# vibhatha/cylon

Hardware: AMD Instinct MI355X
Metric: rows/sec distributed inner-join, 1B×1B int64 keys, at 1/2/4/8 MI355X (higher is better)
Workload: dtype int64 keys / float64 payload; 1 GPU; model=distributed inner join (hash), int64 key + 3 float64 cols, global_batch=1000000000, seq_len=4, parallelism=dp1 (local join), rows_per_relation=1000000000, output_rows=1010151446, key_range=990000000

## Files before the change

cylon_amd/csrc/cylon/kernels/kernel_decls.inc:

```
void row_partition_hash(const ColView *cols, int ncols, int64_t n, uint32_t *h, void *stream);
void hash_to_partition(const uint32_t *h, int64_t n, uint32_t nparts, uint32_t *pid,
                       int64_t *counts, void *stream);
int64_t partition_positions_workspace(int64_t n, uint32_t nparts);
void partition_positions(const uint32_t *pid, int64_t n, uint32_t nparts, int64_t *block_hist,
                         int64_t *pos, int64_t *counts, void *stream);
void scatter_columns(const ColView *in, const MutColView *out, int ncols, const int64_t *pos,
                     int64_t n, void *stream);
void scatter_var_lengths(const ColView &in, const int64_t *pos, int64_t n, int64_t *out_lens
                            , void *stream);
void scatter_var_bytes(const ColView &in, const int64_t *pos, int64_t n,
                       const int64_t *out_offsets, uint8_t *out_bytes, uint8_t *out_valid
                          , void *stream);
void gather_columns(const ColView *in, const MutColView *out, int ncols, const int64_t *idx,
                    int64_t m, void *stream);
void str_to_i64(const ColView &c, int64_t n, int64_t *out, uint8_t *ok, void *stream);
void str_to_f64(const ColView &c, int64_t n, double *out, uint8_t *ok, void *stream);
void i64_to_str_lengths(const int64_t *v, const uint8_t *valid, int64_t n, int64_t *lens, void *stream);
void i64_to_str_write(const int64_t *v, const uint8_t *valid, int64_t n, const int64_t *offs, uint8_t *bytes,
                      void *stream);
void select_var_lengths(const ColView &a, const ColView &b, int b_bcast, const uint8_t *cond, int64_t n,
                        int64_t *out_lens, void *stream);
void select_var_bytes(const ColView &a, const ColView &b, int b_bcast, const uint8_t *cond, int64_t n,
                      const int64_t *out_offsets, uint8_t *out_bytes, uint8_t *out_valid, void *stream);
void gather_var_lengths(const ColView &in, const int64_t *idx, int64_t m, int64_t *out_lens
// ... 106 lines not shown
                    uint64_t *hash = nullptr, bool inv = false);
void words_to_bytes(const int64_t *const *words, int64_t n, int L, uint8_t *bytes, void *stream,
                    const uint64_t *hash = nullptr);
void words_mismatch(const int64_t *const *a, const int64_t *const *b, int W, const uint8_t *va, const uint8_t *vb,
                    int64_t n, uint8_t *bad, int64_t *nbad, void *stream);
void var_to_words(const uint8_t *bytes, const int64_t *offs, int64_t n, int W, int64_t *const *words,
                  uint64_t *hash, int64_t *lens, uint64_t *h2, void *stream, bool text = false,
                  unsigned int *nul = nullptr);
void padded_text_lens(const int64_t *const *words, const uint64_t *hash, int64_t n, int W, int64_t *lens,
                      void *stream);
void words_to_var(const int64_t *const *words, const uint64_t *hash, const int64_t *lens, const int64_t *out_offs,
                  int64_t n, int W, uint8_t *bytes, void *stream, bool text = false);
void var_hash2(const uint8_t *bytes, const int64_t *offs, int64_t n, uint64_t *h1, uint64_t *h2, void *stream,
               bool pack_row = false);
void radix_part_sample(const int64_t *keys, int64_t n, int bits, int64_t stride, uint32_t *hist,
                       const NarrowKeys *nk, void *stream);
void radix_sort_msd_first_pass(const int64_t *keys, int64_t n, int hr, int db1, int db2, uint64_t key_xor,
                               uint64_t sub, int64_t *out, int64_t slot, int64_t *ws, int64_t *counts,
                               unsigned int *overflow, void *stream);
void radix_sort_msd_second_pass(const int64_t *images, int64_t n, int hr, int db1, int db2, uint64_t sub,
                                const int64_t *first_ws, const int64_t *first_counts, int64_t first_slot, int64_t *out,
                                int64_t slot, int64_t *ws, int64_t *counts, unsigned int *overflow, void *stream);
int64_t seg_sort_capacity();
void seg_sort_local(const int64_t *in, const int64_t *counts, int64_t slot, int64_t nparts, const int64_t *out_offs,
                    uint64_t sub, int local_bits, uint64_t out_xor, int64_t *out, void *stream);
void radix_range_rows_pass(const int64_t *keys, int64_t n, uint64_t flip, uint64_t mn, int rshift, int shift,
                           int digit_bits, const uint8_t *const *in, uint8_t *const *out, const int *widths, int ncols,
                           int64_t *ws, void *stream);
void radix_range_part_offsets(const int64_t *keys, int64_t n, uint64_t flip, uint64_t mn, int rshift, int bits,
                              int64_t *offs, void *stream);
int64_t range_join_max_rows();
int range_join_max_shift();
void range_join_count(const int64_t *lkeys, const int64_t *loffs, const int64_t *rkeys, const int64_t *roffs,
                      int64_t nparts, uint64_t flip, uint64_t mn, int rshift, int64_t *counts, int *overflow,
                      void *stream);
void range_join_write(const int64_t *lkeys, const int64_t *loffs, const int64_t *rkeys, const int64_t *roffs,
                      int64_t nparts, uint64_t flip, uint64_t mn, int rshift, const int64_t *out_offs,
                      const uint8_t *const *lin, uint8_t *const *lout, const int *lw, int nlc,
                      const uint8_t *const *rin, uint8_t *const *rout, const int *rw, int nrc, void *stream);
int64_t radix_join_capacity(const int *widths, const uint8_t *const *in, int n, bool match_flags = false, int key_bytes = 8);
constexpr int kRJItemWords = 5;
constexpr int kRJItemPDefer = 1, kRJItemBDefer = 2, kRJItemPEmit = 4, kRJItemBEmit = 8;
struct RJSplit {
  const int64_t *items = nullptr;
  int64_t nitems = 0;
  const uint8_t *skip = nullptr;
  uint8_t *gprobe = nullptr;
  uint8_t *gbuild = nullptr;
};
void radix_join_count(const int64_t *pkeys, const int64_t *poffs, const int64_t *bkeys, const int64_t *boffs,
                      int64_t nparts, int64_t cap, int64_t *counts, int *overflow, void *stream, int64_t pstride = 1,
                      int outer = 0, int64_t pslot = 0, int64_t bslot = 0, const RJSplit *split = nullptr,
                      const int64_t *narrow_base = nullptr);
void radix_join_write(const int64_t *pkeys, const int64_t *poffs, const int64_t *bkeys, const int64_t *boffs,
                      int64_t nparts, int64_t cap, const int64_t *out_offs, const uint8_t *const *pin,
                      uint8_t *const *pout, const int *pw, int npc, const uint8_t *const *bin, uint8_t *const *bout,
                      const int *bw, int nbc, void *stream, int64_t *cursor = nullptr, int64_t out_cap = 0,
                      int *overflow = nullptr, int pkey = -1, int outer = 0, uint8_t *ppres = nullptr,
                      uint8_t *bpres = nullptr, int64_t pslot = 0, int64_t bslot = 0, const RJSplit *split = nullptr,
                      const int64_t *narrow_base = nullptr);
int64_t distinct_estimate_workspace();
double distinct_estimate(const int64_t *keys, int64_t n, uint32_t *regs, void *stream);
int64_t radix_groupby_slots(int nacc);
int radix_groupby_planes(int nacc);
void radix_groupby_agg(const int64_t *keys, const int64_t *offs, int64_t nparts, const RGAccDesc *acc, int nacc,
                       int64_t *okeys, uint64_t *oacc, int64_t n, int64_t *gcount, int *overflow, void *stream);
int64_t radix_quantile_capacity();
void radix_groupby_quantile(const int64_t *keys, const uint8_t *vals, int vwidth, int vkind, const uint8_t *valid,
                            const int64_t *offs, int64_t nparts, int bits, double q, int64_t *okeys, uint64_t *oq,
                            uint64_t *ovalid, int64_t *gcount, int *overflow, void *stream, uint64_t *fused = nullptr,
                            int64_t n = 0);
void radix_groupby_pack(const int64_t *offs, const int64_t *goff, int64_t nparts, const int64_t *okeys,
                        const uint64_t *oacc, int64_t n, int nacc, int64_t *keys_out, uint64_t *acc_out,
                        int64_t ngroups, void *stream);
void radix_sort_rows_pass(const int64_t *keys, int64_t n, int shift, int digit_bits, const uint8_t *const *in,
                          uint8_t *const *out, const int *widths, int ncols, int64_t *ws, void *stream,
                          uint64_t key_xor, uint64_t digit_flip = 0, bool tiles_prescanned = false,
                          const uint16_t *nd_in = nullptr, uint16_t *nd_out = nullptr, int nd_shift = 0,
                          int nd_bits = 0, uint64_t sub = 0, const SortLbArgs *lb = nullptr);
bool radix_sort_lb_eligible(int64_t n, int ncols, const int *widths, const int *dbits, int npass, void *stream);
int64_t radix_sort_lb_workspace(int64_t n);
SortLbArgs radix_sort_lb_args(int64_t *ws, int64_t n, int pass, int npass, void *stream);
bool radix_sort_lb_failed(const int64_t *ws, void *stream);
int64_t radix_sort_prehist_workspace(int64_t n);
uint64_t radix_sort_prehist(const int64_t *keys, int64_t n, uint64_t flip, int64_t *pre_ws, void *stream,
                            uint64_t *img_min = nullptr, uint64_t *img_max = nullptr);
void radix_sort_prehist_fold(const int64_t *pre_ws, int64_t n, int db, int64_t *ws, void *stream, uint64_t sub = 0);
uint64_t varying_bits(const uint64_t *keys, int64_t n, int64_t *ws2, void *stream);
uint64_t sort_keys_varying_bits(const ColView &col, int64_t n, bool desc, uint64_t *out, int64_t *ws2, void *stream);
void setop_row_hash_tiles(const ColView *lcols, const ColView *rcols, int ncols, int64_t nl, int64_t n, uint64_t *h,
                          int bits, int digit_bits, uint16_t *th, void *colsets, void *stream);
int64_t setop_colsets_bytes();
int64_t setop_rows_per_part();
void setop_dedup(const uint64_t *ph, const int64_t *prow, const int64_t *offs, int64_t nparts, int64_t nl, int op,
                 bool keep_last, const ColView *lcols, const ColView *rcols, int ncols, uint8_t *mask, int64_t *exc,
                 int *bad, void *stream);
int64_t semi_join_capacity();
int64_t semi_join_slice_rows();
void semi_join_mark(const int64_t *rkeys, const int64_t *roffs, const int64_t *lkeys, const int64_t *lrow,
                    const int64_t *loffs, int64_t nparts, int anti, uint8_t *mask, int64_t *matched, int *overflow,
                    const int64_t *ipart, const int64_t *islice, int64_t nitems, int64_t *dkeys, int64_t *dmeta,
                    void *stream);
int topk_digit_bits();
int64_t topk_state_words();
int64_t topk_workspace();
void topk_scan(const ColView &col, int64_t n, bool desc, int64_t *ws, void *stream);
void topk_start(int64_t *ws, int64_t k, int ihi, int rhi, void *stream);
void topk_hist(const ColView &col, int64_t n, bool desc, int64_t *ws, int src, int db, void *stream);
void topk_pick(int64_t *ws, int src, int db, void *stream);
void topk_collect(const ColView &col, int64_t n, bool desc, int64_t *ws, uint64_t *sure_img, int64_t *sure_row,
                  int64_t sure_cap, uint64_t *cand_img, int64_t *cand_row, int64_t cand_cap, void *stream);
void narrow_i64(const int64_t *in, int64_t n, int64_t base, uint32_t *out, void *stream);
void widen_u32(const uint32_t *in, int64_t n, int64_t base, int64_t *out, void *stream);
// ... 90 lines not shown
```

cylon_amd/csrc/cylon/kernels/lds_join.hip:

```cpp
#include "radix_common.hpp"

namespace cylon {
namespace hip {

constexpr int kRJBuckets = 4096;

int64_t radix_join_capacity(const int *widths, const uint8_t *const *in, int n, bool match_flags, int key_bytes) {
  int64_t row = key_bytes + 2 + (match_flags ? 1 : 0);
  for (int q = 0; q < n; ++q)
    if (in[q]) row += widths[q];
  int64_t cap = kRJRowArea / row;
  cap = std::min<int64_t>(cap, kRJMaxRows);
  return cap & ~int64_t(7);
}

__device__ __forceinline__ uint32_t rj_bucket(int64_t k) {
  return (uint32_t)hashing::fmix64((uint64_t)k) & (kRJBuckets - 1);
}
__device__ __forceinline__ uint32_t rj_bucket(uint32_t k) { return hashing::fmix32(k) & (kRJBuckets - 1); }

constexpr int kRJRowsPerThread = kRJMaxRows / kRJThreads;
static_assert(kRJRowsPerThread * kRJThreads == kRJMaxRows, "build rows per thread");
constexpr int kRJProbeRounds = 1;

// ... 460 lines not shown
          if (pc.n > MAXP) {
            const int64_t lo = s0 + (int64_t)u * kWave + owner;
            for (int q = MAXP; q < pc.n; ++q)
              stw<W8>(pc.out[q], o, pc.width[q], q == pkey ? kw : ldw<W8>(pc.in[q], lo, pc.width[q]));
          }
          if ((OJ & kOJProbe) && r < 0) {
#pragma unroll
            for (int q = 0; q < MAXB + 1; ++q)
              if (q < bo.n) stw<W8>(bo.out[q], o, bo.width[q], 0ull);
            for (int q = MAXB + 1; q < bo.n; ++q) stw<W8>(bo.out[q], o, bo.width[q], 0ull);
          } else {
#pragma unroll
            for (int q = 0; q < MAXB + 1; ++q)
              if (q < bo.n)
                stw<W8>(bo.out[q], o, bo.width[q],
                        bo.lds_off[q] < 0 ? kw : ldw<W8>(area + bo.lds_off[q], r, bo.width[q]));
            for (int q = MAXB + 1; q < bo.n; ++q)
              stw<W8>(bo.out[q], o, bo.width[q],
                      bo.lds_off[q] < 0 ? kw : ldw<W8>(area + bo.lds_off[q], r, bo.width[q]));
          }
          if (OJ & kOJProbe) bpres[o] = r >= 0 ? 1 : 0;
          if (OJ & kOJBuild) ppres[o] = 1;
        }
      }
      base += wsum;
    }
    if ((OJ & kOJBuild) && !bdefer) {
      __syncthreads();
      int64_t at = ubase;
      for (int i0 = 0; i0 < nr; i0 += kRJThreads) {
        const int i = i0 + (int)threadIdx.x;
        const uint32_t um = (i < nr && !flg[i]) ? 1u : 0u;
        const uint32_t ex = rp_block_exscan<kRJWaves>(um, wtot);
        uint32_t tot = 0;
#pragma unroll
        for (int w = 0; w < kRJWaves; ++w) tot += wtot[w];
        if (um) {
          const int64_t o = at + ex;
          const int r = perm[i];
          const uint64_t kw = key_value(skeys[i]);
          for (int q = 0; q < pc.n; ++q) stw<W8>(pc.out[q], o, pc.width[q], q == pkey ? kw : 0ull);
          for (int q = 0; q < bo.n; ++q)
            stw<W8>(bo.out[q], o, bo.width[q], bo.lds_off[q] < 0 ? kw : ldw<W8>(area + bo.lds_off[q], r, bo.width[q]));
          ppres[o] = 0;
          if (OJ & kOJProbe) bpres[o] = 1;
        }
        at += tot;
        __syncthreads();
      }
    }
  }
}

static int rj_grid(int64_t nparts) { return (int)std::min<int64_t>(nparts, kNumCUs * 8); }

void radix_join_count(const int64_t *pkeys, const int64_t *poffs, const int64_t *bkeys, const int64_t *boffs,
                      int64_t nparts, int64_t cap, int64_t *counts, int *overflow, void *stream, int64_t pstride,
                      int outer, int64_t pslot, int64_t bslot, const RJSplit *split, const int64_t *narrow_base) {
  CYLON_CHECK(cap > 0 && cap <= kRJMaxRows, Code::Invalid, "radix join capacity " << cap);
  CYLON_CHECK(pstride >= 1, Code::Invalid, "partition stride " << pstride);
  CYLON_CHECK(outer >= 0 && outer <= 3, Code::Invalid, "radix join outer mode " << outer);
  hipStream_t s = as_stream(stream);
  HIP_CHECK(hipMemsetAsync(overflow, 0, sizeof(int), s));
  const int64_t *items = split ? split->items : nullptr;
  const int64_t nitems = items ? split->nitems : 0;
  const uint8_t *skip = split ? split->skip : nullptr;
  const int64_t nsample = items ? nitems : (nparts + pstride - 1) / pstride;
  if (nsample == 0) return;
  const dim3 grid((unsigned)std::max<int64_t>(1, std::min<int64_t>(nsample, kNumCUs * 12)));
  switch (outer) {
    case 0:
      if (narrow_base)
        hipLaunchKernelGGL((k_rj_count<0, true>), grid, dim3(kRCThreads), 0, s, pkeys, poffs, bkeys, boffs, nparts,
                           (int)cap, pstride, counts, overflow, pslot, bslot, items, nitems, skip);
      else
        hipLaunchKernelGGL((k_rj_count<0, false>), grid, dim3(kRCThreads), 0, s, pkeys, poffs, bkeys, boffs, nparts,
                           (int)cap, pstride, counts, overflow, pslot, bslot, items, nitems, skip);
      break;
    case 1:
      if (narrow_base)
        hipLaunchKernelGGL((k_rj_count<1, true>), grid, dim3(kRCThreads), 0, s, pkeys, poffs, bkeys, boffs, nparts,
                           (int)cap, pstride, counts, overflow, pslot, bslot, items, nitems, skip);
      else
        hipLaunchKernelGGL((k_rj_count<1, false>), grid, dim3(kRCThreads), 0, s, pkeys, poffs, bkeys, boffs, nparts,
                           (int)cap, pstride, counts, overflow, pslot, bslot, items, nitems, skip);
      break;
    case 2:
      if (narrow_base)
        hipLaunchKernelGGL((k_rj_count<2, true>), grid, dim3(kRCThreads), 0, s, pkeys, poffs, bkeys, boffs, nparts,
                           (int)cap, pstride, counts, overflow, pslot, bslot, items, nitems, skip);
      else
        hipLaunchKernelGGL((k_rj_count<2, false>), grid, dim3(kRCThreads), 0, s, pkeys, poffs, bkeys, boffs, nparts,
                           (int)cap, pstride, counts, overflow, pslot, bslot, items, nitems, skip);
      break;
    default:
      if (narrow_base)
        hipLaunchKernelGGL((k_rj_count<3, true>), grid, dim3(kRCThreads), 0, s, pkeys, poffs, bkeys, boffs, nparts,
                           (int)cap, pstride, counts, overflow, pslot, bslot, items, nitems, skip);
      else
        hipLaunchKernelGGL((k_rj_count<3, false>), grid, dim3(kRCThreads), 0, s, pkeys, poffs, bkeys, boffs, nparts,
                           (int)cap, pstride, counts, overflow, pslot, bslot, items, nitems, skip);
  }
  HIP_LAUNCH_CHECK();
}

template <bool W8, bool DMA, int OJ>
static void rj_write_launch(dim3 grid, hipStream_t s, const int64_t *pk, const int64_t *poffs, const int64_t *bk,
                            const int64_t *boffs, int64_t nparts, int cap, const int64_t *out_offs, const ColSet &pc,
                            const ColSet &bs, const BuildOut &bo, unsigned long long *cur, int64_t out_cap,
                            int *overflow, int pkey, uint8_t *ppres, uint8_t *bpres,
                            int64_t pslot, int64_t bslot, const RJSplit &sp, const int64_t *nb) {
  if (nb)
    hipLaunchKernelGGL((k_rj_write<4, 3, W8, DMA, OJ, true>), grid, dim3(kRJThreads), 0, s, pk, poffs, bk, boffs, nparts,
                       cap, out_offs, pc, bs, bo, cur, out_cap, overflow, pkey, ppres, bpres, pslot, bslot, sp.items,
                       sp.nitems, sp.skip, sp.gprobe, sp.gbuild, nb);
  else
    hipLaunchKernelGGL((k_rj_write<4, 3, W8, DMA, OJ, false>), grid, dim3(kRJThreads), 0, s, pk, poffs, bk, boffs,
                       nparts, cap, out_offs, pc, bs, bo, cur, out_cap, overflow, pkey, ppres, bpres, pslot, bslot,
                       sp.items, sp.nitems, sp.skip, sp.gprobe, sp.gbuild, nb);
}

void radix_join_write(const int64_t *pkeys, const int64_t *poffs, const int64_t *bkeys, const int64_t *boffs,
                      int64_t nparts, int64_t cap, const int64_t *out_offs, const uint8_t *const *pin,
                      uint8_t *const *pout, const int *pw, int npc, const uint8_t *const *bin, uint8_t *const *bout,
                      const int *bw, int nbc, void *stream, int64_t *cursor, int64_t out_cap, int *overflow, int pkey,
                      int outer, uint8_t *ppres, uint8_t *bpres, int64_t pslot, int64_t bslot,
                      const RJSplit *split, const int64_t *narrow_base) {
  CYLON_CHECK(pkey >= -1 && pkey < npc, Code::Invalid, "radix join probe key column " << pkey);
  CYLON_CHECK(npc <= kMaxFusedCols && nbc <= kMaxFusedCols, Code::Invalid, "too many columns");
  CYLON_CHECK(out_offs != nullptr || (cursor != nullptr && overflow != nullptr), Code::Invalid,
              "radix join write: needs partition offsets or an output cursor");
  CYLON_CHECK(outer >= 0 && outer <= 3, Code::Invalid, "radix join outer mode " << outer);
  CYLON_CHECK(!(outer & kOJProbe) || bpres, Code::Invalid, "radix join: probe-preserving mode needs build presence");
  CYLON_CHECK(!(outer & kOJBuild) || ppres, Code::Invalid, "radix join: build-preserving mode needs probe presence");
  const RJSplit sp = split ? *split : RJSplit{};
  CYLON_CHECK(sp.nitems == 0 || (out_offs == nullptr && sp.items), Code::Invalid,
              "radix join write: split items need the cursor mode");
  if (sp.nitems + nparts == 0) return;
  const int kbytes = narrow_base ? 4 : 8;
  CYLON_CHECK(cap > 0 && cap <= radix_join_capacity(bw, bin, nbc, outer & kOJBuild, kbytes), Code::Invalid,
              "radix join capacity " << cap);
  ColSet pc, bs;
  BuildOut bo;
  pc.n = npc;
  bs.n = 0;
  bo.n = nbc;
  bool w8 = true;
  for (int q = 0; q < kMaxFusedCols; ++q) {
    pc.in[q] = q < npc ? pin[q] : nullptr;
    pc.out[q] = q < npc ? pout[q] : nullptr;
    pc.width[q] = q < npc ? pw[q] : 8;
    bs.in[q] = nullptr;
    bs.out[q] = nullptr;
    bs.width[q] = 8;
    bo.out[q] = q < nbc ? bout[q] : nullptr;
    bo.width[q] = q < nbc ? bw[q] : 8;
    bo.lds_off[q] = -1;
    if (q < npc) w8 &= pw[q] == 8;
    if (q < nbc) w8 &= bw[q] == 8;
  }
  int64_t off = (kbytes + 2) * cap;
  for (int q = 0; q < nbc; ++q)
    if (bin[q]) {
      bo.lds_off[q] = (int)off;
      off += cap * bw[q];
      bs.in[bs.n] = bin[q];
      bs.width[bs.n++] = bw[q];
    }
  bo.match_off = (int)off;
  if (outer & kOJBuild) off += cap;
  CYLON_CHECK(off <= kRJRowArea, Code::Invalid, "radix join LDS rows " << off);
  hipStream_t s = as_stream(stream);
  unsigned long long *cur = reinterpret_cast<unsigned long long *>(cursor);
  const dim3 grid(rj_grid(nparts + sp.nitems));
  const bool dma = w8;
  const int ci = (int)cap;
#define RJW(W8_, DMA_, OJ_)                                                                                        \
  rj_write_launch<W8_, DMA_, OJ_>(grid, s, pkeys, poffs, bkeys, boffs, nparts, ci, out_offs, pc, bs, bo, cur, out_cap, \
                                  overflow, pkey, ppres, bpres, pslot, bslot, sp, narrow_base)
  if (outer == 0) {
    if (dma) RJW(true, true, 0);
    else if (w8) RJW(true, false, 0);
    else RJW(false, false, 0);
  } else if (outer == 1) {
    if (dma) RJW(true, true, 1);
    else RJW(false, false, 1);
  } else if (outer == 2) {
    if (dma) RJW(true, true, 2);
    else RJW(false, false, 2);
  } else {
    if (dma) RJW(true, true, 3);
    else RJW(false, false, 3);
  }
#undef RJW
  HIP_LAUNCH_CHECK();
}


void preload_lds_join() { preload_code(reinterpret_cast<const void *>(&(k_rj_count<0, false>))); }

}
}
```

cylon_amd/csrc/cylon/ops/join_radix.cpp:

```cpp
#include "cylon/knobs.hpp"
#include <algorithm>
#include <array>
#include <cmath>
#include <cstdlib>

#include "join_internal.hpp"
#include "radix_sizing.hpp"
#include "../trace.hpp"

namespace cylon {
namespace ops {

int64_t radix_join_min_rows() {
  return knobs::Int("RADIX_JOIN_MIN_ROWS", int64_t(1) << 22);
}

bool radix_eligible(const TablePtr &t) {
  int slots = 1;
  for (const auto &c : t->columns()) {
    const int w = c.type.width();
    if (c.is_var() || c.type.kind() == ValueKind::FIXED_BYTES || !(w == 1 || w == 2 || w == 4 || w == 8) ||
        c.data.element_size() != w)
      return false;
    slots += 1 + (c.nullable() ? 1 : 0);
// ... 189 lines not shown
  p.cap4 = capacity(4);
  p.cap8 = capacity(8);
  p.narrow = narrow;
  p.split_rows = split_rows_of(p.cap());
  const int64_t nb = std::min(p.nl, p.nr);
  if (pre_bits >= 0) {
    p.set_bits(pre_bits);
    return p;
  }
  p.set_bits(radix_extra_bits(sizing::partition_bits(nb, p.cap())));
  if (p.narrow && p.bits == 0) {
    p = p.without_narrowing();
    p.set_bits(radix_extra_bits(sizing::partition_bits(nb, p.cap())));
  }
  return p;
}

struct RadixJoinIn {
  const Exec &ex;
  const TablePtr &left, &right;
  const JoinConfig &cfg;
  JoinSink *sink;
  const PrePartition *pre;
};

struct Narrowing {
  at::Tensor bad;
  at::Tensor base_src;
  hip::NarrowKeys nk;
};

struct SkewMasks {
  at::Tensor bcnt, pcnt, heavy, mid, sums;
  int64_t cap = 0;
};

static SkewMasks skew_masks(const RadixJoinPlan &plan, const RadixSide &Bs, const RadixSide &Ps) {
  SkewMasks k;
  k.cap = plan.cap();
  const int64_t nparts = plan.nparts, np_rows = plan.build_left ? plan.nr : plan.nl;
  k.bcnt = part_counts(Bs, nparts);
  k.pcnt = part_counts(Ps, nparts);
  k.heavy = at::logical_or(k.bcnt > plan.split_rows, k.pcnt > 2 * plan.pch);
  k.mid = at::logical_and(k.heavy.logical_not(),
                          at::logical_or(k.pcnt > 4 * (np_rows + nparts - 1) / nparts + 1024, k.bcnt > 4 * plan.bmean + 1024));
  k.sums = at::stack({k.heavy.sum(), k.mid.sum()});
  return k;
}

struct Partitioned {
  RadixSide L, R;
  bool released = false;
  SkewMasks sk;
};

static bool fail(bool released, const char *why) {
  CYLON_CHECK(!released, Code::ExecutionError,
              "radix join with a released (retain = false) input could not complete: " << why);
  return false;
}

static void drop_slots_of_skewed_sides(const RadixJoinIn &in, const RadixJoinPlan &plan, const at::Tensor &lk,
                                       const at::Tensor &rk, const hip::NarrowKeys *nkp, int64_t &sl, int64_t &sr) {
  const Exec &ex = in.ex;
  auto sample = [&](const at::Tensor &k, int64_t rows, at::Tensor &h, int64_t &stride) {
    stride = std::max<int64_t>(1, rows >> 20);
    h = at::empty({plan.nparts}, ex.opts(at::kInt));
    hip::radix_part_sample(ptr<int64_t>(k), rows, plan.bits, stride, reinterpret_cast<uint32_t *>(h.data_ptr<int>()),
                           nkp, ex.stream);
  };
  at::Tensor hl, hr;
  int64_t stl = 1, str = 1;
  sample(lk, plan.nl, hl, stl);
  sample(rk, plan.nr, hr, str);
  at::Tensor mx = at::stack({hl.max(), hr.max()}).cpu();
  auto hot = [&](int64_t m, int64_t rows, int64_t stride) {
    const double mean = (double)((rows + stride - 1) / stride) / (double)plan.nparts;
    return (double)m > 4.0 * mean + 32.0;
  };
  if (sl && hot(mx[0].item<int>(), plan.nl, stl)) sl = 0;
  if (sr && hot(mx[1].item<int>(), plan.nr, str)) sr = 0;
  if (!sl || !sr) trace::add_counter("join.radix.sampled_skew_sides", (sl ? 0 : 1) + (sr ? 0 : 1));
}

static Partitioned partition_sides(const RadixJoinIn &in, RadixJoinPlan &plan, at::Tensor &lk, at::Tensor &rk,
                                   const Narrowing &nw) {
  const Exec &ex = in.ex;
  const TablePtr &left = in.left, &right = in.right;
  const int bits = plan.bits;
  Partitioned out;
  RadixSide &L = out.L, &R = out.R;
  const bool rel_l = !left->IsRetain() && !in.sink, rel_r = !right->IsRetain() && !in.sink;
  const bool narrow = plan.narrow;
  at::Tensor r_outside;
  if (rel_l && narrow) {
    auto mm = at::aminmax(rk);
    const at::Tensor base = nw.base_src - (int64_t(1) << 31);
    r_outside = at::logical_or(std::get<0>(mm) < base, (std::get<1>(mm) - base) > (int64_t)0xffffffffll).to(at::kInt);
  }
  auto release_if_done = [&](const TablePtr &t, at::Tensor &key, const RadixSide &s, const at::Tensor *outside) {
    at::Tensor z = at::zeros({1}, ex.opts(at::kInt));
    std::vector<at::Tensor> flags{s.slot ? s.overflow.slice(0, 0, 1) : z, narrow ? nw.bad : z};
    if (outside) flags.push_back(outside->defined() ? outside->reshape({1}) : z);
    if (at::cat(flags).sum().item<int>() != 0) return;
    t->ReleaseIfNotRetained();
    key = at::Tensor();
    trace::add_counter("join.radix.released_inputs", 1);
    out.released = true;
  };
  CYLON_PHASE("join.radix.partition", ex.device);
  const hip::NarrowKeys *nkp = narrow ? &nw.nk : nullptr;
  const bool slot_on = knobs::Flag("RJ_SLOT", true);
  int64_t sl = slot_on ? plan.slot_l : 0, sr = slot_on ? plan.slot_r : 0;
  if ((sl || sr) && std::max(plan.nl, plan.nr) >= (int64_t(1) << 24) && (!in.sink || in.sink->sample_skew))
    drop_slots_of_skewed_sides(in, plan, lk, rk, nkp, sl, sr);
  L = radix_partition(ex, left, lk, bits, nullptr, sl, nkp);
  if (rel_l) release_if_done(left, lk, L, &r_outside);
  R = radix_partition(ex, right, rk, bits, nullptr, sr, nkp);
  if (rel_r) release_if_done(right, rk, R, nullptr);
  if (!(L.slot || R.slot || narrow)) return out;
  at::Tensor z = at::zeros({}, ex.opts(at::kInt));
  out.sk = skew_masks(plan, plan.build_left ? L : R, plan.build_left ? R : L);
  at::Tensor f = at::cat({at::stack({L.slot ? L.overflow[0] : z, R.slot ? R.overflow[0] : z,
                                     narrow ? nw.bad[0] : z}).to(at::kLong),
                          out.sk.sums}).cpu();
  bool redo = f[2].item<int64_t>() != 0;
  if (redo) {
    trace::add_counter("join.radix.narrow_fallback", 1);
    plan = plan.without_narrowing();
    nkp = nullptr;
    L = radix_partition(ex, left, lk, bits, nullptr, slot_on ? plan.slot_l : 0);
    R = radix_partition(ex, right, rk, bits, nullptr, slot_on ? plan.slot_r : 0);
    if (L.slot || R.slot)
      f = at::stack({L.slot ? L.overflow[0] : z, R.slot ? R.overflow[0] : z, z}).to(at::kLong).cpu();
  }
  if (f[0].item<int64_t>()) {
    trace::add_counter("join.radix.slot_overflow", 1);
    L = radix_partition(ex, left, lk, bits, nullptr, 0, nkp);
    redo = true;
  }
  if (f[1].item<int64_t>()) {
    trace::add_counter("join.radix.slot_overflow", 1);
    R = radix_partition(ex, right, rk, bits, nullptr, 0, nkp);
    redo = true;
  }
  if (redo) out.sk = SkewMasks();
  else out.sk.sums = f.slice(0, 3, 5);
  trace::add_counter("join.radix.slot_sides", (L.slot ? 1 : 0) + (R.slot ? 1 : 0));
  if (plan.narrow) trace::add_counter("join.radix.narrow_keys", 1);
  return out;
}

struct SplitWork {
  int64_t nheavy = 0, nmid = 0, nitems = 0, nemits = 0;
  int64_t emit_bound = 0;
  at::Tensor skip, skip_sample, items_d, emits_d, gprobe, gbuild, mid_items;
  hip::RJSplit main, emit;
};

static void split_items(const RadixJoinPlan &plan, const int64_t *h, int64_t nheavy, std::vector<int64_t> &items,
                        std::vector<int64_t> &emits, int64_t &emit_bound) {
  const int oj = plan.oj;
  const int64_t split_rows = plan.split_rows, pch = plan.pch;
  std::vector<std::array<int64_t, hip::kRJItemWords>> work;
  for (int64_t i = 0; i < nheavy; ++i) {
    const int64_t lb0 = h[4 * i], nl0 = h[4 * i + 1], rb0 = h[4 * i + 2], nr0 = h[4 * i + 3];
    const int64_t nbc = std::max<int64_t>(1, (nr0 + split_rows - 1) / split_rows);
    const int64_t npc = nl0 > 2 * pch ? (nl0 + pch - 1) / pch : 1;
    const bool pdef = (oj & 1) && nbc > 1, bdef = (oj & 2) && npc > 1;
    const int64_t fl = (pdef ? hip::kRJItemPDefer : 0) | (bdef ? hip::kRJItemBDefer : 0);
    for (int64_t bc = 0; bc < nbc; ++bc)
      for (int64_t pc = 0; pc < npc; ++pc) {
        const int64_t b0 = nr0 * bc / nbc, b1 = nr0 * (bc + 1) / nbc, p0 = nl0 * pc / npc, p1 = nl0 * (pc + 1) / npc;
        if (b1 > b0 || p1 > p0) work.push_back({lb0 + p0, p1 - p0, rb0 + b0, b1 - b0, fl});
      }
    if (pdef) {
      for (int64_t pc = 0; pc < npc; ++pc)
        emits.insert(emits.end(), {lb0 + nl0 * pc / npc, nl0 * (pc + 1) / npc - nl0 * pc / npc, 0, 0,
                                   (int64_t)hip::kRJItemPEmit});
      emit_bound += nl0;
    }
    if (bdef) {
      for (int64_t bc = 0; bc < nbc; ++bc)
// ... 187 lines not shown
      for (const auto &col : t->columns())
        proto.emplace_back(prefix + col.name, col.type, 0, col.data, at::Tensor(),
                           col.nullable() || may_null ? col.data : at::Tensor());
    };
    add(in.left, in.cfg.GetLeftTablePrefix(), left_may_null(in.cfg.GetType()));
    add(in.right, in.cfg.GetRightTablePrefix(), right_may_null(in.cfg.GetType()));
    o.off = in.sink->reserve(ex, rows, proto);
    o.lcols.assign(in.sink->cols.begin(), in.sink->cols.begin() + nlc);
    o.rcols.assign(in.sink->cols.begin() + nlc, in.sink->cols.end());
  } else {
    auto add = [&](const TablePtr &t, const std::string &prefix, int shared_col, std::vector<Column> &cols) {
      for (int c = 0; c < t->Columns(); ++c)
        cols.push_back(make_fixed_column(prefix + t->column(c).name, t->column(c).type, c == shared_col ? 0 : rows,
                                         ex.device, t->column(c).nullable()));
    };
    add(in.left, in.cfg.GetLeftTablePrefix(), share.on && plan.build_left ? share.kl : -1, o.lcols);
    add(in.right, in.cfg.GetRightTablePrefix(), share.on && !plan.build_left ? share.kr : -1, o.rcols);
  }
  auto word_outs = [&](const RadixSide &sd) {
    std::vector<at::Tensor> w;
    for (size_t i = 0; i < sd.vwords.size(); ++i) w.push_back(ex.empty_i64(std::max<int64_t>(rows, 1)));
    return w;
  };
  o.lwords = word_outs(pt.L);
  o.rwords = word_outs(pt.R);
  if (plan.oj & 2) o.ppres = ex.empty_u8(std::max<int64_t>(rows, 1));
  if (plan.oj & 1) o.bpres = ex.empty_u8(std::max<int64_t>(rows, 1));
}

static void write_output(const RadixJoinIn &in, const JoinLaunch &jl, const Partitioned &pt, const SharedKey &share,
                         const SplitWork &w, JoinOutput &o, int64_t rows, const int64_t *offs, int64_t *cursor) {
  const RadixJoinPlan &plan = jl.plan;
  const RadixSide &P = jl.P, &B = jl.B;
  const bool build_left = plan.build_left;
  RadixCols lc = radix_cols(in.left, &pt.L, &o.lcols, o.off, &o.lwords);
  RadixCols rc = radix_cols(in.right, &pt.R, &o.rcols, o.off, &o.rwords);
  RadixCols &pc = build_left ? rc : lc, &bc = build_left ? lc : rc;
  if (share.on) {
    const TablePtr &bt = build_left ? in.left : in.right;
    const int bkc = build_left ? share.kl : share.kr;
    int q = 0;
    for (int c = 0; c < bkc; ++c) q += 1 + (bt->column(c).nullable() && B.vwords.empty());
    bc.in.erase(bc.in.begin() + q);
    bc.out.erase(bc.out.begin() + q);
    bc.w.erase(bc.w.begin() + q);
  }
  int pkey = -1;
  for (size_t q = 0; q < pc.in.size(); ++q)
    if (!pc.in[q]) {
      pc.in[q] = reinterpret_cast<const uint8_t *>(P.keys.data_ptr());
      if (pkey < 0) pkey = (int)q;
    }
  auto launch = [&](int64_t np, const int64_t *out_offs, const hip::RJSplit &sp) {
    hip::radix_join_write(kptr(P.keys), ptr<int64_t>(P.offs), kptr(B.keys), ptr<int64_t>(B.offs), np, plan.cap(),
                          out_offs, pc.in.data(), pc.out.data(), pc.w.data(), (int)pc.in.size(), bc.in.data(),
                          bc.out.data(), bc.w.data(), (int)bc.in.size(), jl.ex.stream, cursor, rows,
                          jl.overflow.data_ptr<int>(), pkey, plan.oj,
                          o.ppres.defined() ? o.ppres.data_ptr<uint8_t>() : nullptr,
                          o.bpres.defined() ? o.bpres.data_ptr<uint8_t>() : nullptr, P.slot, B.slot, &sp, jl.nbase);
  };
  launch(plan.nparts, offs, w.main);
  if (w.nemits > 0) launch(0, nullptr, w.emit);
}

static bool allocate_and_write(const RadixJoinIn &in, const JoinLaunch &jl, const Partitioned &pt,
                               const SharedKey &share, const SplitWork &w, JoinOutput &o) {
  const Exec &ex = in.ex;
  JoinSink *sink = in.sink;
  const at::Tensor &overflow = jl.overflow;
  int64_t &m = o.m;
  if (o.stride == 1) {
    allocate_output(in, jl.plan, pt, share, m, o);
    if (m > 0) write_output(in, jl, pt, share, w, o, m, ptr<int64_t>(o.out_offs), nullptr);
    return true;
  }
  at::Tensor cursor = at::zeros({1}, ex.opts(at::kLong));
  overflow.zero_();
  allocate_output(in, jl.plan, pt, share, o.alloc, o);
  write_output(in, jl, pt, share, w, o, o.alloc, nullptr, ptr<int64_t>(cursor));
  at::Tensor res = at::cat({cursor, overflow.to(at::kLong)}).cpu();
  m = res[0].item<int64_t>();
  const int64_t flags = res[1].item<int64_t>();
  if (flags & 1) {
    if (sink) sink->size = o.off;
    trace::add_counter("join.radix.overflow_fallback", 1);
    return fail(pt.released, "overflow");
  }
  if (flags & 2) {
    trace::add_counter("join.radix.estimate_rerun", 1);
    if (sink) sink->size = o.off;
    cursor.zero_();
    overflow.zero_();
    if (w.gprobe.defined()) w.gprobe.zero_();
    if (w.gbuild.defined()) w.gbuild.zero_();
    allocate_output(in, jl.plan, pt, share, m, o);
    write_output(in, jl, pt, share, w, o, m, nullptr, ptr<int64_t>(cursor));
    CYLON_CHECK(at::cat({cursor, overflow.to(at::kLong)}).cpu().equal(at::tensor({m, (int64_t)0})),
                Code::ExecutionError, "radix join: exact rerun did not match its own count");
  } else if (sink) {
    sink->size = o.off + m;
  }
  if (!sink) {
    for (auto &c : o.lcols)
      if (c.length > 0) c = c.slice(0, m);
    for (auto &c : o.rcols)
      if (c.length > 0) c = c.slice(0, m);
  }
  return true;
}

static TablePtr finish_columns(const RadixJoinIn &in, const RadixJoinPlan &plan, const Partitioned &pt,
                               const SharedKey &share, JoinOutput &o) {
// ... 89 lines not shown
```

Measured before the change: 25.46 billion rows/s.

## Add specialized exact-shape radix join write kernel with cached probe results

Adds a templated write kernel for inner joins whose columns are all 8 bytes wide, with up to three payload columns per side. It caches packed probe results (first slot, contiguity bit and match count) for the first rounds and uses a DPP wave scan to distribute matches across lanes. It also prefetches the next probe key and its payload so each match is emitted with direct 64-bit stores instead of generic width-dispatched stores. The goal is to cut repeated probing and generic column handling in the write phase, at the cost of more code paths and register pressure. A flag disables it after a narrow-key fallback.

```diff
diff --git a/cylon_amd/csrc/cylon/kernels/kernel_decls.inc b/cylon_amd/csrc/cylon/kernels/kernel_decls.inc
--- a/cylon_amd/csrc/cylon/kernels/kernel_decls.inc
+++ b/cylon_amd/csrc/cylon/kernels/kernel_decls.inc
@@ -182,13 +182,13 @@
                       int64_t nparts, int64_t cap, int64_t *counts, int *overflow, void *stream, int64_t pstride = 1,
                       int outer = 0, int64_t pslot = 0, int64_t bslot = 0, const RJSplit *split = nullptr,
                       const int64_t *narrow_base = nullptr);
-void radix_join_write(const int64_t *pkeys, const int64_t *poffs, const int64_t *bkeys, const int64_t *boffs,
+bool radix_join_write(const int64_t *pkeys, const int64_t *poffs, const int64_t *bkeys, const int64_t *boffs,
                       int64_t nparts, int64_t cap, const int64_t *out_offs, const uint8_t *const *pin,
                       uint8_t *const *pout, const int *pw, int npc, const uint8_t *const *bin, uint8_t *const *bout,
                       const int *bw, int nbc, void *stream, int64_t *cursor = nullptr, int64_t out_cap = 0,
                       int *overflow = nullptr, int pkey = -1, int outer = 0, uint8_t *ppres = nullptr,
                       uint8_t *bpres = nullptr, int64_t pslot = 0, int64_t bslot = 0, const RJSplit *split = nullptr,
-                      const int64_t *narrow_base = nullptr);
+                      const int64_t *narrow_base = nullptr, bool exact_ok = true);
 int64_t distinct_estimate_workspace();
 double distinct_estimate(const int64_t *keys, int64_t n, uint32_t *regs, void *stream);
 int64_t radix_groupby_slots(int nacc);
diff --git a/cylon_amd/csrc/cylon/kernels/lds_join.hip b/cylon_amd/csrc/cylon/kernels/lds_join.hip
--- a/cylon_amd/csrc/cylon/kernels/lds_join.hip
+++ b/cylon_amd/csrc/cylon/kernels/lds_join.hip
@@ -536,6 +536,224 @@
   }
 }
 
+constexpr int kRJExactCols = 3;
+struct ExactCols {
+  const uint64_t *pin[kRJExactCols];
+  uint64_t *pout[kRJExactCols];
+  uint64_t *kout;
+  const uint8_t *bin[kRJExactCols];
+  uint64_t *bout[kRJExactCols];
+};
+
+constexpr int kRJKeptRounds = 8;
+constexpr uint32_t kRJPureBit = 1u << 13, kRJSlotMask = kRJPureBit - 1;
+constexpr int kRJCountShift = 14;
+static_assert(kRJMaxRows <= (int)kRJPureBit && kRJMaxRows < (1 << (32 - kRJCountShift)), "packed probe result");
+
+template <class KT>
+__device__ __forceinline__ uint32_t rj_probe_pack(const uint16_t *bst, const KT *skeys, KT k) {
+  const uint32_t b = rj_bucket(k);
+  uint32_t i0 = 0, last = 0, mc = 0;
+  for (uint32_t i = bst[b], e = bst[b + 1]; i < e; ++i)
+    if (skeys[i] == k) {
+      if (mc == 0) i0 = i;
+      last = i;
+      ++mc;
+    }
+  return i0 | (mc > 0 && last - i0 + 1 == mc ? kRJPureBit : 0u) | (mc << kRJCountShift);
+}
+
+template <int CTRL, int ROWS>
+__device__ __forceinline__ uint32_t rj_dpp_add(uint32_t x) {
+  return x + (uint32_t)__builtin_amdgcn_update_dpp(0, (int)x, CTRL, ROWS, 0xF, false);
+}
+__device__ __forceinline__ uint32_t rj_wave_incscan(uint32_t x) {
+  x = rj_dpp_add<0x111, 0xF>(x);
+  x = rj_dpp_add<0x112, 0xF>(x);
+  x = rj_dpp_add<0x114, 0xF>(x);
+  x = rj_dpp_add<0x118, 0xF>(x);
+  x = rj_dpp_add<0x142, 0xA>(x);
+  x = rj_dpp_add<0x143, 0xC>(x);
+  return x;
+}
+
+template <int NP, int NB, bool NK>
+__global__ __launch_bounds__(kRJThreads, 4) void k_rj_write_exact(
+    const int64_t *__restrict__ pkeys0, const int64_t *__restrict__ poffs, const int64_t *__restrict__ bkeys0,
+    const int64_t *__restrict__ boffs, int64_t nparts, int cap, const int64_t *__restrict__ out_offs, ExactCols xc,
+    unsigned long long *__restrict__ cursor, int64_t out_cap, int *__restrict__ overflow, int64_t pslot,
+    int64_t bslot, const int64_t *__restrict__ narrow_base) {
+  static_assert(NP >= 1 && NP <= kRJExactCols && NB >= 1 && NB <= kRJExactCols, "exact shape");
+  using KT = typename std::conditional<NK, uint32_t, int64_t>::type;
+  const KT *__restrict__ pkeys = reinterpret_cast<const KT *>(pkeys0);
+  const KT *__restrict__ bkeys = reinterpret_cast<const KT *>(bkeys0);
+  const uint64_t nbase = NK ? (uint64_t)narrow_base[0] - (uint64_t(1) << 31) : 0;
+  __shared__ __attribute__((aligned(16))) uint16_t bst[kRJBuckets + 8];
+  __shared__ __attribute__((aligned(16))) uint8_t area[kRJRowArea];
+  __shared__ uint32_t wtot[kRJWaves];
+  __shared__ int64_t sclaim;
+  KT *skeys = reinterpret_cast<KT *>(area);
+  uint16_t *perm = reinterpret_cast<uint16_t *>(area + sizeof(KT) * (int64_t)cap);
+  const uint64_t *bcol = reinterpret_cast<const uint64_t *>(area + (int64_t)(sizeof(KT) + 2) * cap);
+  const int lane = lane_id();
+  const int wave = threadIdx.x / kWave;
+  for (int64_t p = blockIdx.x; p < nparts; p += gridDim.x) {
+    int64_t rb, nr, lb, nl;
+    part_span(boffs, bslot, p, rb, nr);
+    part_span(poffs, pslot, p, lb, nl);
+    if (nr > cap && out_offs == nullptr && threadIdx.x == 0) atomicOr(overflow, 1);
+    if (nr == 0 || nl == 0 || nr > cap) continue;
+    const int64_t per = (nl + kRJWaves - 1) / kRJWaves;
+    const int64_t s0 = lb + std::min<int64_t>(nl, wave * per);
+    const int64_t s1 = lb + std::min<int64_t>(nl, (wave + 1) * per);
+    KT pk0 = 0;
+    uint64_t pv0[NP] = {};
+    if (s0 + lane < s1) {
+      pk0 = pkeys[s0 + lane];
+#pragma unroll
+      for (int q = 0; q < NP; ++q) pv0[q] = xc.pin[q][s0 + lane];
+    }
+    __syncthreads();
+    for (int s = threadIdx.x; s < kRJBuckets / 2; s += blockDim.x) reinterpret_cast<uint32_t *>(bst)[s] = 0;
+    rj_dma(reinterpret_cast<const uint8_t *>(bkeys + rb), nr * (int)sizeof(KT), area, wave, lane);
+#pragma unroll
+    for (int j = 0; j < NB; ++j)
+      rj_dma(xc.bin[j] + rb * 8, nr * 8, area + (int64_t)(sizeof(KT) + 2) * cap + (int64_t)j * cap * 8, wave, lane);
+    asm volatile("s_waitcnt vmcnt(0)" ::: "memory");
+    __syncthreads();
+    KT bk[kRJRowsPerThread];
+#pragma unroll
+    for (int i = 0; i < kRJRowsPerThread; ++i) {
+      const int r = threadIdx.x + i * kRJThreads;
+      if (r < nr) bk[i] = skeys[r];
+    }
+    uint32_t rk[kRJRowsPerThread];
+#pragma unroll
+    for (int i = 0; i < kRJRowsPerThread; ++i)
+      if (threadIdx.x + i * kRJThreads < nr) rk[i] = rj_claim(bst, rj_bucket(bk[i]));
+    __syncthreads();
+    rj_scan_buckets(bst, wtot);
+    __syncthreads();
+#pragma unroll
+    for (int i = 0; i < kRJRowsPerThread; ++i) {
+      const int r = threadIdx.x + i * kRJThreads;
+      if (r < nr) {
+        const uint32_t pos = bst[rj_bucket(bk[i])] + rk[i];
+        skeys[pos] = bk[i];
+        perm[pos] = (uint16_t)r;
+      }
+    }
+    __syncthreads();
+    uint32_t kept[kRJKeptRounds];
+#pragma unroll
+    for (int r = 0; r < kRJKeptRounds; ++r) kept[r] = 0;
+    if (s0 + lane < s1) kept[0] = rj_probe_pack<KT>(bst, skeys, pk0);
+#pragma unroll
+    for (int r = 1; r < kRJKeptRounds; r += 2) {
+      const int64_t l = s0 + r * kWave + lane;
+      if (s0 + r * kWave < s1) {
+        const bool a = l < s1, b = r + 1 < kRJKeptRounds && l + kWave < s1;
+        KT ka = 0, kb = 0;
+        if (a) ka = pkeys[l];
+        if (b) kb = pkeys[l + kWave];
+        if (a) kept[r] = rj_probe_pack<KT>(bst, skeys, ka);
+        if (b) kept[r + 1 < kRJKeptRounds ? r + 1 : r] = rj_probe_pack<KT>(bst, skeys, kb);
+      }
+    }
+    uint32_t c = 0;
+#pragma unroll
+    for (int r = 0; r < kRJKeptRounds; ++r) c += kept[r] >> kRJCountShift;
+    {
+      int64_t l = s0 + (int64_t)kRJKeptRounds * kWave + lane;
+      for (; l + kWave < s1; l += 2 * kWave) {
+        const KT ka = pkeys[l], kb = pkeys[l + kWave];
+        c += rj_count_mark<0, KT>(bst, skeys, ka, nullptr) + rj_count_mark<0, KT>(bst, skeys, kb, nullptr);
+      }
+      if (l < s1) c += rj_count_mark<0, KT>(bst, skeys, pkeys[l], nullptr);
+    }
+    for (int d = kWave / 2; d > 0; d >>= 1) c += __shfl_xor(c, d, kWave);
+    if (lane == 0) wtot[wave] = c;
+    __syncthreads();
+    int64_t base = out_offs ? out_offs[p] : 0;
+    if (out_offs == nullptr) {
+      if (threadIdx.x == 0) {
+        unsigned long long tot = 0;
+        for (int w = 0; w < kRJWaves; ++w) tot += wtot[w];
+        const unsigned long long at = tot ? atomicAdd(cursor, tot) : 0ull;
+        const bool fits = at + tot <= (unsigned long long)out_cap;
+        if (!fits) atomicOr(overflow, 2);
+        sclaim = fits ? (int64_t)at : -1;
+      }
+      __syncthreads();
+      base = sclaim;
+      if (base < 0) continue;
+    }
+    for (int w = 0; w < wave; ++w) base += wtot[w];
+    KT kn = pk0;
+    uint64_t vn[NP];
+#pragma unroll
+    for (int q = 0; q < NP; ++q) vn[q] = pv0[q];
+    for (int u = 0; s0 + (int64_t)u * kWave < s1; ++u) {
+      const int64_t l = s0 + (int64_t)u * kWave + lane;
+      const KT k = kn;
+      uint64_t v[NP];
+#pragma unroll
+      for (int q = 0; q < NP; ++q) v[q] = vn[q];
+      if (l + kWave < s1) {
+        kn = pkeys[l + kWave];
+#pragma unroll
+        for (int q = 0; q < NP; ++q) vn[q] = xc.pin[q][l + kWave];
+      }
+      uint32_t word = 0;
+      if (u < kRJKeptRounds) {
+#pragma unroll
+        for (int r = 0; r < kRJKeptRounds; ++r) word = u == r ? kept[r] : word;
+      } else if (l < s1) {
+        word = rj_probe_pack<KT>(bst, skeys, k);
+      }
+      const uint32_t inc = rj_wave_incscan(word >> kRJCountShift);
+      const uint32_t wsum = __builtin_amdgcn_readlane(inc, kWave - 1);
+      for (uint32_t t0 = 0; t0 < wsum; t0 += kWave) {
+        const uint32_t so = t0 + lane;
+        int owner = 0;
+#pragma unroll
+        for (int step = kWave / 2; step >= 1; step >>= 1) {
+          const uint32_t ic = __shfl(inc, owner + step - 1, kWave);
+          if (ic <= so) owner += step;
+        }
+        const uint32_t ow = __shfl(word, owner, kWave);
+        const uint32_t j = so + (ow >> kRJCountShift) - __shfl(inc, owner, kWave);
+        const KT ko = rj_shfl_key(k, owner);
+        const uint64_t kw = NK ? nbase + (uint64_t)ko : (uint64_t)ko;
+        uint64_t vo[NP];
+#pragma unroll
+        for (int q = 0; q < NP; ++q) vo[q] = (uint64_t)rj_shfl64((int64_t)v[q], owner);
+        if (so < wsum) {
+          uint32_t slot = (ow & kRJSlotMask) + j;
+          if (!(ow & kRJPureBit)) {
+            uint32_t i = ow & kRJSlotMask, m = 0;
+            const uint32_t e = bst[rj_bucket(ko) + 1];
+            for (; i < e; ++i)
+              if (skeys[i] == ko && m++ == j) break;
+            slot = i;
+          }
+          const uint32_t r = perm[slot];
+          uint64_t bv[NB];
+#pragma unroll
+          for (int q = 0; q < NB; ++q) bv[q] = bcol[(int64_t)q * cap + r];
+          const int64_t o = base + so;
+          xc.kout[o] = kw;
+#pragma unroll
+          for (int q = 0; q < NP; ++q) xc.pout[q][o] = vo[q];
+#pragma unroll
+          for (int q = 0; q < NB; ++q) xc.bout[q][o] = bv[q];
+        }
+      }
+      base += wsum;
+    }
+  }
+}
+
 static int rj_grid(int64_t nparts) { return (int)std::min<int64_t>(nparts, kNumCUs * 8); }
 
 void radix_join_count(const int64_t *pkeys, const int64_t *poffs, const int64_t *bkeys, const int64_t *boffs,
@@ -604,12 +822,25 @@
                        sp.items, sp.nitems, sp.skip, sp.gprobe, sp.gbuild, nb);
 }
 
-void radix_join_write(const int64_t *pkeys, const int64_t *poffs, const int64_t *bkeys, const int64_t *boffs,
+template <int NP, int NB>
+static void rj_write_exact_launch(dim3 grid, hipStream_t s, const int64_t *pk, const int64_t *poffs, const int64_t *bk,
+                                  const int64_t *boffs, int64_t nparts, int cap, const int64_t *out_offs,
+                                  const ExactCols &xc, unsigned long long *cur, int64_t out_cap, int *overflow,
+                                  int64_t pslot, int64_t bslot, const int64_t *nb) {
+  if (nb)
+    hipLaunchKernelGGL((k_rj_write_exact<NP, NB, true>), grid, dim3(kRJThreads), 0, s, pk, poffs, bk, boffs, nparts, cap,
+                       out_offs, xc, cur, out_cap, overflow, pslot, bslot, nb);
+  else
+    hipLaunchKernelGGL((k_rj_write_exact<NP, NB, false>), grid, dim3(kRJThreads), 0, s, pk, poffs, bk, boffs, nparts,
+                       cap, out_offs, xc, cur, out_cap, overflow, pslot, bslot, nb);
+}
+
+bool radix_join_write(const int64_t *pkeys, const int64_t *poffs, const int64_t *bkeys, const int64_t *boffs,
                       int64_t nparts, int64_t cap, const int64_t *out_offs, const uint8_t *const *pin,
                       uint8_t *const *pout, const int *pw, int npc, const uint8_t *const *bin, uint8_t *const *bout,
                       const int *bw, int nbc, void *stream, int64_t *cursor, int64_t out_cap, int *overflow, int pkey,
                       int outer, uint8_t *ppres, uint8_t *bpres, int64_t pslot, int64_t bslot,
-                      const RJSplit *split, const int64_t *narrow_base) {
+                      const RJSplit *split, const int64_t *narrow_base, bool exact_ok) {
   CYLON_CHECK(pkey >= -1 && pkey < npc, Code::Invalid, "radix join probe key column " << pkey);
   CYLON_CHECK(npc <= kMaxFusedCols && nbc <= kMaxFusedCols, Code::Invalid, "too many columns");
   CYLON_CHECK(out_offs != nullptr || (cursor != nullptr && overflow != nullptr), Code::Invalid,
@@ -620,7 +851,7 @@
   const RJSplit sp = split ? *split : RJSplit{};
   CYLON_CHECK(sp.nitems == 0 || (out_offs == nullptr && sp.items), Code::Invalid,
               "radix join write: split items need the cursor mode");
-  if (sp.nitems + nparts == 0) return;
+  if (sp.nitems + nparts == 0) return false;
   const int kbytes = narrow_base ? 4 : 8;
   CYLON_CHECK(cap > 0 && cap <= radix_join_capacity(bw, bin, nbc, outer & kOJBuild, kbytes), Code::Invalid,
               "radix join capacity " << cap);
@@ -659,6 +890,32 @@
   const dim3 grid(rj_grid(nparts + sp.nitems));
   const bool dma = w8;
   const int ci = (int)cap;
+  if (exact_ok && outer == 0 && w8 && sp.nitems == 0 && sp.skip == nullptr && pkey == 0 && npc >= 2 &&
+      npc <= 1 + kRJExactCols && nbc >= 1 && nbc <= kRJExactCols && bs.n == nbc) {
+    ExactCols xc = {};
+    xc.kout = reinterpret_cast<uint64_t *>(pout[0]);
+    for (int q = 1; q < npc; ++q) {
+      xc.pin[q - 1] = reinterpret_cast<const uint64_t *>(pin[q]);
+      xc.pout[q - 1] = reinterpret_cast<uint64_t *>(pout[q]);
+    }
+    for (int q = 0; q < nbc; ++q) {
+      xc.bin[q] = bin[q];
+      xc.bout[q] = reinterpret_cast<uint64_t *>(bout[q]);
+    }
+#define RJX(NP_, NB_)                                                                                            \
+  case (NP_) * 4 + (NB_):                                                                                        \
+    rj_write_exact_launch<NP_, NB_>(grid, s, pkeys, poffs, bkeys, boffs, nparts, ci, out_offs, xc, cur, out_cap, \
+                                    overflow, pslot, bslot, narrow_base);                                        \
+    break
+    switch ((npc - 1) * 4 + nbc) {
+      RJX(1, 1); RJX(1, 2); RJX(1, 3);
+      RJX(2, 1); RJX(2, 2); RJX(2, 3);
+      RJX(3, 1); RJX(3, 2); RJX(3, 3);
+    }
+#undef RJX
+    HIP_LAUNCH_CHECK();
+    return true;
+  }
 #define RJW(W8_, DMA_, OJ_)                                                                                        \
   rj_write_launch<W8_, DMA_, OJ_>(grid, s, pkeys, poffs, bkeys, boffs, nparts, ci, out_offs, pc, bs, bo, cur, out_cap, \
                                   overflow, pkey, ppres, bpres, pslot, bslot, sp, narrow_base)
@@ -678,6 +935,7 @@
   }
 #undef RJW
   HIP_LAUNCH_CHECK();
+  return false;
 }
 
 
diff --git a/cylon_amd/csrc/cylon/ops/join_radix.cpp b/cylon_amd/csrc/cylon/ops/join_radix.cpp
--- a/cylon_amd/csrc/cylon/ops/join_radix.cpp
+++ b/cylon_amd/csrc/cylon/ops/join_radix.cpp
@@ -265,6 +265,7 @@
   RadixSide L, R;
   bool released = false;
   SkewMasks sk;
+  bool widened = false;
 };
 
 static bool fail(bool released, const char *why) {
@@ -342,6 +343,7 @@
     trace::add_counter("join.radix.narrow_fallback", 1);
     plan = plan.without_narrowing();
     nkp = nullptr;
+    out.widened = true;
     L = radix_partition(ex, left, lk, bits, nullptr, slot_on ? plan.slot_l : 0);
     R = radix_partition(ex, right, rk, bits, nullptr, slot_on ? plan.slot_r : 0);
     if (L.slot || R.slot)
@@ -635,12 +637,15 @@
       if (pkey < 0) pkey = (int)q;
     }
   auto launch = [&](int64_t np, const int64_t *out_offs, const hip::RJSplit &sp) {
-    hip::radix_join_write(kptr(P.keys), ptr<int64_t>(P.offs), kptr(B.keys), ptr<int64_t>(B.offs), np, plan.cap(),
+    const bool exact =
+        hip::radix_join_write(kptr(P.keys), ptr<int64_t>(P.offs), kptr(B.keys), ptr<int64_t>(B.offs), np, plan.cap(),
                           out_offs, pc.in.data(), pc.out.data(), pc.w.data(), (int)pc.in.size(), bc.in.data(),
                           bc.out.data(), bc.w.data(), (int)bc.in.size(), jl.ex.stream, cursor, rows,
                           jl.overflow.data_ptr<int>(), pkey, plan.oj,
                           o.ppres.defined() ? o.ppres.data_ptr<uint8_t>() : nullptr,
-                          o.bpres.defined() ? o.bpres.data_ptr<uint8_t>() : nullptr, P.slot, B.slot, &sp, jl.nbase);
+                          o.bpres.defined() ? o.bpres.data_ptr<uint8_t>() : nullptr, P.slot, B.slot, &sp, jl.nbase,
+                          !pt.widened);
+    if (exact) trace::add_counter("join.radix.write_exact", 1);
   };
   launch(plan.nparts, offs, w.main);
   if (w.nemits > 0) launch(0, nullptr, w.emit);
```

Result: faster. 26.84 billion rows/s (median of 6 runs) (+5.4%).
